# kmkolasinski/tfrecords-reader

Hardware: AMD Instinct MI355X
Metric: GiB/s + examples/s device-resident TFRecord->Feature decode, 1/2/4/8 GPU (higher is better)
Workload: dtype u8; 1 GPU; C4 directory (configs[4]) of 256 files, C1-shaped (int64 label + 12 B bytes_list id) records, 524288 +-50 % per file (default_rng(1000+f)), spec CRC-32C; this rank's LPT share (256 files) resident in HBM; records_per_gpu=134295581, framed_bytes_per_gpu=7906235019, parallelism=file-sharded x1 (LPT by bytes, no collective on the data path), batches_per_gpu=4, batch_bytes_max=1976558779, streams=2, tpl_groups_missed=0

## Files before the change

### tfrecords-reader_amd/csrc/tfrg_capi.cpp

```cpp
#include <hip/hip_runtime.h>
#include <stdlib.h>
#include <string.h>

#include <algorithm>
#include <map>
#include <numeric>
#include <string>
#include <unordered_map>
#include <vector>

#include "../../include/tfrg.h"
#include "crc32c.h"
#include "tfrg_internal.h"

namespace tfrg {
void set_error(const std::string& s);

#define HIP_TRY(expr)                                                              \
  do {                                                                             \
    hipError_t e_ = (expr);                                                        \
    if (e_ != hipSuccess) {                                                        \
      set_error(std::string(#expr) + ": " + hipGetErrorString(e_));               \
      return TFRG_E_HIP;                                                           \
    }                                                                              \
// ... 12 lines not shown
    }
    size_t want = bytes < 256 ? 256 : bytes;
    want = (want + 4095) & ~(size_t)4095;
    hipError_t e = hipMalloc(&p, want);
    if (e == hipSuccess) cap = want;
    return e;
  }
  void release() {
    if (p) (void)hipFree(p);
    p = nullptr;
    cap = 0;
  }
  template <class T>
  T* as() const {
    return reinterpret_cast<T*>(p);
  }
};

constexpr uint32_t kMissCap = 1u << 16;

const CrcTables& crc_tables() {
  static const CrcTables T = [] {
    CrcTables t;
    crc_make_tables(&t);
    return t;
  }();
  return T;
}

}

using namespace tfrg;

struct Offsets {
  const uint64_t* s64 = nullptr;
  const uint64_t* e64 = nullptr;
  const uint32_t* s32 = nullptr;
  const uint32_t* e32 = nullptr;
  uint32_t first = 0;
  uint32_t mode = kOffU64;
};

struct tfrg_ctx {
  int device = 0;
  hipStream_t own_stream = nullptr;
  hipStream_t last_stream = nullptr;
  uint32_t lane_max = 2048;
  uint32_t wave_stage = 0xffffffffu;
  uint64_t record_bound = 0;
  uint64_t call_bound = 0;
  int num_cus = 256;
  uint32_t cu_lds = 65536;
  int tpl_stage = 1;
  DBuf crc_tab, consts;
  DBuf ht, key_hash, key_off, key_blob, key_slot, slot_kind, key_w, krec;
  uint32_t n_keys = 0, n_slots = 0, ht_mask = 0;
  DBuf in_bytes, in_start, in_end;
  DBuf status, aux, verdict, order, count, loc, rs, slot_base, totals, kind_totals;
  DBuf ident;
  size_t ident_n = 0;
  DBuf i64, f32, b_off, b_len, big_list, slow_list, miss, info, tsum, crc_rec, crc_base, crc_part;
  DBuf dq, dq_cnt;
  DBuf lmask, rlist;
  DBuf bdata, boff64, blb, bbig;
  bool materialized = false;
  bool tsum_dirty = true;
  uint32_t info_slot = 0;
  bool info_clean = false;
  uint32_t n = 0;
  uint64_t cap_hint = 0;
  hipEvent_t order_ev = nullptr;
  uint64_t nbytes = 0;
  uint64_t cap_i64 = 0, cap_f32 = 0, cap_b = 0;
  bool have_result = false;
  bool rs_complete = false;
  std::unordered_map<std::string, uint32_t> key_id;
  std::vector<int32_t> key_slot_h;
  DBuf tpl;
  uint32_t n_tpl = 0;
  uint32_t tpl_w = 0;
  size_t tpl_img_off = 0;
  uint32_t tpl_img_words = 0;
  uint32_t tpl_tab_words = 0;
  std::vector<uint32_t> tpl_h;
  bool tpl_learned = false;
  bool tpl_full = false;
  uint32_t tpl_frames = 0;
  bool tpl_on = true;
  std::vector<uint8_t> slot_kind_h;
  DBuf spec;
  std::vector<uint32_t> spec_h;
  bool have_spec = false;
  bool spec_on = true;
  bool profiling = false;
  bool have_events = false;
  hipEvent_t ev[kNumStages + 1] = {};
  uint64_t hint_i64 = 0, hint_f32 = 0, hint_b = 0;
  bool hinted = false;
  bool no_hints = false;
  uint64_t hint_reruns = 0;
  bool optimistic_on = true;
  bool walk_beside = true;
  uint32_t walk_blocks = 0;
  bool no_quiet = false;
  bool opt_pending = false;
  bool ord_const = false;
  bool len_const = false;
  std::vector<uint32_t> const_len;
  uint32_t last_implicit = 0;
  bool last_aux_zero = false;
  uint32_t* info_pin = nullptr;
  bool cols_complete = false;
  bool mat_pending = false;
  struct LastCall {
    const uint8_t* d_bytes;
    uint64_t nbytes;
    uint64_t cap_in;
    uint64_t bound;
    uint32_t n, flags;
    hipStream_t st;
  } last{};
  Offsets last_off{};
  uint32_t poison[4] = {0xffffffffu, 0xffffffffu, 0xffffffffu, 0xffffffffu};
};

extern "C" {

int tfrg_ctx_create(int device, tfrg_ctx** out) {
  *out = nullptr;
  int ndev = 0;
  HIP_TRY(hipGetDeviceCount(&ndev));
  if (device < 0 || device >= ndev) {
    set_error("bad device index");
    return TFRG_E_ARG;
  }
  HIP_TRY(hipSetDevice(device));
  tfrg_ctx* c = new tfrg_ctx();
  c->device = device;
  if (const char* e = getenv("TFRG_TEMPLATES")) c->tpl_on = atoi(e) != 0;
  if (const char* e = getenv("TFRG_SPEC")) c->spec_on = atoi(e) != 0;
  if (const char* e = getenv("TFRG_TPL_STAGE")) c->tpl_stage = atoi(e);
  if (const char* e = getenv("TFRG_OPTIMISTIC")) c->optimistic_on = atoi(e) != 0;
  if (const char* e = getenv("TFRG_WALK_BESIDE")) c->walk_beside = atoi(e) != 0;
  if (const char* e = getenv("TFRG_WALK_BLOCKS")) c->walk_blocks = (uint32_t)atoi(e);
  if (const char* e = getenv("TFRG_DEBUG_POISON_LOC")) {
    char* q = const_cast<char*>(e);
    for (int i = 0; i < 4 && *q; ++i) {
      c->poison[i] = (uint32_t)strtoul(q, &q, 10);
      while (*q == ',' || *q == ' ') ++q;
    }
  }
  hipDeviceProp_t prop;
  if (hipGetDeviceProperties(&prop, device) == hipSuccess) {
    c->num_cus = prop.multiProcessorCount;
    if (prop.maxSharedMemoryPerMultiProcessor) c->cu_lds = (uint32_t)prop.maxSharedMemoryPerMultiProcessor;
  }
  if (hipStreamCreateWithFlags(&c->own_stream, hipStreamNonBlocking) != hipSuccess) {
    delete c;
    set_error("hipStreamCreate failed");
    return TFRG_E_HIP;
  }
  if (hipHostMalloc(reinterpret_cast<void**>(&c->info_pin), (kInfoCount + 8) * 4) != hipSuccess) {
    (void)hipStreamDestroy(c->own_stream);
    delete c;
    set_error("hipHostMalloc failed");
    return TFRG_E_NOMEM;
  }
  std::vector<uint32_t> tab(kCrcTabWords), cst(128);
  CrcTables T;
  crc_make_tables(&T);
  memcpy(tab.data(), T.t, 4096);
  uint32_t M[4][256];
  crc_make_mul_tables(gf_xpow8(1024), M);
  memcpy(tab.data() + 1024, M, 4096);
  memcpy(tab.data() + 2048, T.t, 8192);
  memcpy(tab.data() + 4096, T.t, 16384);
  for (int e = 0; e < 256; ++e)
    for (int col = 0; col < 47; ++col) tab[8192 + e * 64 + col] = T.t[(col + 1) & 15][e];
  crc_make_mul_tables(gf_xpow8(2048), M);
  memcpy(tab.data() + 24576, M, 4096);
  crc_make_mul_tables(gf_xpow8(4096), M);
  memcpy(tab.data() + 25600, M, 4096);
  for (int k = 0; k < 24; ++k) {
    crc_make_mul_tables(gf_xpow8(1024ull << k), M);
    memcpy(tab.data() + 26624 + k * 1024, M, 4096);
  }
  for (int l = 0; l < 64; ++l) cst[l] = gf_xpow8(16ull * l);
  for (int z = 0; z < 16; ++z) cst[64 + z] = gf_xpow8_inv((uint64_t)z);
  for (int k = 0; k < 32; ++k) cst[96 + k] = gf_xpow8(1024ull << k);
  if (c->crc_tab.ensure(tab.size() * 4) != hipSuccess || c->consts.ensure(cst.size() * 4) != hipSuccess ||
      hipMemcpy(c->crc_tab.p, tab.data(), tab.size() * 4, hipMemcpyHostToDevice) != hipSuccess ||
      hipMemcpy(c->consts.p, cst.data(), cst.size() * 4, hipMemcpyHostToDevice) != hipSuccess) {
    set_error("constant upload failed");
    tfrg_ctx_destroy(c);
// ... 837 lines not shown
    if (!n) HIP_TRY(hipMemsetAsync(c->boff64.p, 0, 8, st));
  }
  if (!S || !n) HIP_TRY(hipMemsetAsync(c->kind_totals.p, 0, 32, st));

  DevBatch b;
  b.bytes = d_bytes;
  b.nbytes = nbytes;
  b.start = off.s64;
  b.end = off.e64;
  b.start32 = off.s32;
  b.end32 = off.e32;
  b.first = off.first;
  b.omode = off.mode;
  b.n = n;
  b.flags = flags;
  DevOut o;
  o.status = c->status.as<int32_t>();
  o.aux = c->aux.as<int64_t>();
  o.verdict = c->verdict.as<uint8_t>();
  o.order = c->order.as<uint16_t>();
  o.count = c->count.as<uint32_t>();
  o.loc = c->loc.as<uint2>();
  o.rs = c->rs.as<uint32_t>();
  o.slot_base = c->slot_base.as<uint64_t>();
  o.totals = c->totals.as<uint32_t>();
  o.kind_totals = c->kind_totals.as<uint64_t>();
  o.i64 = c->i64.as<int64_t>();
  o.f32 = c->f32.as<uint32_t>();
  o.b_off = c->b_off.as<uint32_t>();
  o.b_len = c->b_len.as<uint32_t>();
  o.cap_i64 = cap_i64;
  o.cap_f32 = cap_f32;
  o.cap_b = cap_b;
  o.big_list = c->big_list.as<uint32_t>();
  o.miss = c->miss.as<uint32_t>();
  o.miss_cap = kMissCap;
  o.info = info_cur;
  o.info_next = c->info.as<uint32_t>() + (islot ^ 1u) * kInfoCount;
  o.tsum = c->tsum.as<uint32_t>();
  o.tile_stride = tile_stride;
  o.spine_lb = reinterpret_cast<uint64_t*>(o.tsum + (size_t)S * tile_stride);
  o.n_chunks = n_chunks;
  o.irr = o.tsum + (size_t)S * tile_stride + 2ull * S * n_chunks;
  o.slow_list = c->slow_list.as<uint32_t>();
  o.crc_rec = c->crc_rec.as<uint32_t>();
  o.crc_base = c->crc_base.as<uint64_t>();
  o.crc_part = c->crc_part.as<uint64_t>();
  o.lmask = c->lmask.as<uint64_t>();
  o.rlist = c->rlist.as<uint32_t>();
  LaunchCfg cfg;
  cfg.num_cus = c->num_cus;
  cfg.tpl_cu_lds = c->tpl_stage ? c->cu_lds : 0u;
  cfg.tpl_stage_any = c->tpl_stage == 2;
  cfg.lean = c->tpl_on && c->n_tpl;
  cfg.tpl_full = cfg.lean && c->tpl_full;
  cfg.tpl_unchecked = cfg.lean && (c->tpl_frames & 2u) != 0;
  cfg.spec_h = c->spec_h.empty() ? nullptr : c->spec_h.data();
  const uint64_t lane_blocks = (n + 255) / 256;
  const uint64_t lane_cap = (uint64_t)c->num_cus * 8;
  cfg.lane_grid = (int)(lane_blocks < 1 ? 1 : (lane_blocks < lane_cap ? lane_blocks : lane_cap));
  const uint64_t wave_cap = (uint64_t)c->num_cus * 4;
  const uint64_t wave_blocks = (n + 3) / 4;
  cfg.wave_grid = (int)(wave_blocks < 1 ? 1 : (wave_blocks < wave_cap ? wave_blocks : wave_cap));
  cfg.lane_max = c->lane_max;
  cfg.wave_stage = c->wave_stage;
  memcpy(cfg.poison, c->poison, sizeof(cfg.poison));
  cfg.optimistic = c->optimistic_on && !c->no_quiet && c->poison[0] == 0xffffffffu;
  cfg.walk_beside = c->walk_beside;
  cfg.walk_blocks = c->walk_blocks;
  cfg.ran_optimistic = false;
  cfg.ran_quiet_big = false;
  cfg.ord_const = c->ord_const;
  cfg.len_const = c->len_const && !mat;
  cfg.implicit = 0;
  const uint64_t bound = c->call_bound ? c->call_bound : c->record_bound;
  c->call_bound = 0;
  c->last = tfrg_ctx::LastCall{d_bytes, nbytes, cap_in, bound, n, flags, st};
  c->last_off = off;
  o.dq = nullptr;
  o.dq_cnt = nullptr;
  o.dq_blocks = 0;
  cfg.body_count = false;
  if (n && (bound == 0 || bound > c->lane_max)) {
    uint64_t blocks = nbytes >> 18;
    blocks = blocks < 16 ? 16 : (blocks > (1u << 16) ? (1u << 16) : blocks);
    const size_t qb = (size_t)blocks * 64u * kDeferK * 16u, cb = (size_t)blocks * 64u;
    if ((c->dq.cap < qb || c->dq_cnt.cap < cb) && c->last_stream) HIP_TRY(hipStreamSynchronize(c->last_stream));
    if (c->dq.ensure(qb) || c->dq_cnt.ensure(cb)) {
      set_error("device allocation failed (deferred bodies)");
      return TFRG_E_NOMEM;
    }
    o.dq = c->dq.as<uint4>();
    o.dq_cnt = c->dq_cnt.as<uint8_t>();
    o.dq_blocks = (uint32_t)blocks;
    cfg.body_count = true;
  }
  if (n) {
    hipEvent_t* ev = nullptr;
    if (c->profiling) {
      if (!c->have_events) {
        for (auto& e : c->ev) HIP_TRY(hipEventCreate(&e));
        c->have_events = true;
      }
      ev = c->ev;
    }
    hipError_t e = launch_decode(b, schema_view(c), o, cfg, c->crc_tab.as<uint32_t>(), c->consts.as<uint32_t>(), st, ev);
// ... 280 lines not shown
```

### tfrecords-reader_amd/csrc/tfrg_internal.h

```cpp
#pragma once
#include <stdint.h>
#include <hip/hip_runtime.h>

namespace tfrg {

struct DevSchema {
  uint32_t n_keys;
  uint32_t n_slots;
  uint32_t ht_mask;
  const uint32_t* ht;
  const uint32_t* key_hash;
  const uint32_t* key_off;
  const uint8_t* key_blob;
  const int32_t* key_slot;
  const uint8_t* slot_kind;
  const uint32_t* key_w;
  const uint32_t* krec;
  const uint32_t* tpl;
  const uint32_t* tpl_img;
  uint32_t tpl_img_words;
  uint32_t tpl_tab_words;
  uint32_t n_tpl;
  uint32_t tpl_w;
  const uint32_t* spec;
};

constexpr uint32_t kTplMaxL = 240, kTplMaxEntries = 16;
constexpr uint32_t kLtMaxW = 64;
constexpr uint32_t kLeanMaxSlots = 16;
constexpr uint32_t kLtL = 0, kLtNe = 1, kLtCrcw = 2, kLtChain = 3, kLtK = 4, kLtAbsent = 5, kLtFrame = 6, kLtEnt = 8,
                   kLtWin = kLtEnt + 4 * kTplMaxEntries, kLtSlot = kLtWin + 3 * kLtMaxW,
                   kLtWords = kLtSlot + 3 * kLeanMaxSlots;
constexpr uint32_t kCrcTabWords = 51200;

constexpr uint32_t kLiPtabWords = 4 * 256;
constexpr uint32_t kTplMaxLane = 32;
constexpr uint32_t kLiHdr = 8, kLiSlotQ = kLiHdr, kLiLut = kLiSlotQ + kLeanMaxSlots,
                   kLiLutWords = (kTplMaxL + 1 + 3) / 4, kLiTpl = (kLiLut + kLiLutWords + 3) & ~3u;
constexpr uint32_t kLiQValue = 1u << 16, kLiQSingle = 1u << 17;
__host__ __device__ constexpr uint32_t kLiTw(uint32_t W) { return 4 + 3 * W + 4 * kLeanMaxSlots; }
constexpr uint32_t kLiMaxWords = (65536u - 32768u - 512u) / 4u;

struct LeanTgt {
  uint16_t* ord;
  uint32_t* cnt;
  uint2* loc;
  uint32_t* rs;
  void* v1;
  uint32_t* v2;
  uint32_t lim;
  uint32_t kind;
  uint32_t pad[2];
};
struct LeanArgs {
  uint32_t n_tpl;
  uint32_t lane_max;
  uint32_t* tsum;
  uint32_t n_slots;
  uint32_t tile_stride;
  uint32_t img_words;
  uint32_t gpw;
  uint32_t bsplit;
  uint32_t gsplit;
  const uint8_t* finish;
  uint32_t implicit;
  uint32_t tab_words;
  uint32_t cu_lds;
  uint32_t stage_any;
  uint32_t nocrc;
  uint32_t strict;
  uint32_t uframes;
  LeanTgt tg[kLeanMaxSlots];
};

enum KeyRec : uint32_t { kKrHash = 0, kKrLen, kKrW0, kKrW1, kKrSlot1, kKrSlot2, kKrSlot3, kKrFlags, kKrWords };
constexpr uint32_t kLdsMaxKeys = 256;
constexpr uint32_t kLdsMaxHt = 1024;

__host__ __device__ inline uint32_t key_hash_words(uint32_t n, uint32_t w0, uint32_t w1) {
  const uint32_t a = (w0 ^ (w0 >> 11) ^ (n << 17)) & 0xffffffu;
  const uint32_t b = (w1 ^ (w1 >> 13) ^ (n << 7)) & 0xffffffu;
#if defined(__HIP_DEVICE_COMPILE__)
  uint32_t p0, p1;
  asm("v_mul_u32_u24 %0, %1, %2" : "=v"(p0) : "v"(a), "v"(0x9E3779u));
  asm("v_mul_u32_u24 %0, %1, %2" : "=v"(p1) : "v"(b), "v"(0x85EBCBu));
  uint32_t h = p0 ^ p1;
#else
  uint32_t h = a * 0x9E3779u;
  h ^= b * 0x85EBCBu;
#endif
  return h ^ (h >> 15);
}

enum OffMode : uint32_t { kOffU64 = 0, kOffU32 = 1, kOffEnds = 2 };

struct DevBatch {
  const uint8_t* bytes;
  uint64_t nbytes;
  const uint64_t* start;
  const uint64_t* end;
  const uint32_t* start32;
  const uint32_t* end32;
  uint32_t first;
  uint32_t omode;
  uint32_t n;
  uint32_t flags;
};

#if defined(__HIPCC__)
__device__ __forceinline__ uint64_t rec_end(const DevBatch& B, uint32_t r) {
  return B.omode == kOffU64 ? B.end[r] : (uint64_t)B.end32[r];
}
__device__ __forceinline__ uint64_t rec_start(const DevBatch& B, uint32_t r) {
  if (B.omode == kOffU64) return B.start[r];
  if (B.omode == kOffU32) return B.start32[r];
  return r ? (uint64_t)B.end32[r - 1] : (uint64_t)B.first;
}
#endif

enum InfoIdx : uint32_t {
  kInfoErrors = 0,
// ... 70 lines not shown
  uint64_t* lmask;
  uint32_t* rlist;
};

constexpr uint32_t kTileShift = 8;
constexpr uint32_t kTileRecs = 1u << kTileShift;
constexpr uint32_t kSpineChunkShift = 12;

constexpr uint32_t kFlagPayloadOnly = 1u;
constexpr uint32_t kFlagSpecVarint = 2u;
constexpr uint32_t kFlagNoCrc = 4u;
constexpr uint32_t kFlagStrictCrc = 8u;
constexpr uint32_t kFlagMaterializeBytes = 16u;


struct DevBytes {
  const uint8_t* in;
  uint64_t in_readable;
  const uint32_t* b_off;
  const uint32_t* b_len;
  const uint64_t* kind_totals;
  uint64_t* offsets;
  uint64_t offsets_cap;
  uint8_t* data;
  uint64_t data_cap;
  uint64_t* lb;
  uint32_t* ticket;
  uint32_t* big_count;
  uint32_t* big_list;
  uint32_t* overflow;
};
hipError_t launch_materialize(const DevBytes& d, int num_cus, hipStream_t st);
uint64_t materialize_lb_words(uint64_t cap_b);

struct LaunchCfg {
  int num_cus;
  bool lean;
  bool tpl_full;
  bool tpl_unchecked;
  const uint32_t* spec_h;
  int lane_grid;
  int wave_grid;
  uint32_t lane_max;
  uint32_t wave_stage;
  bool body_count;
  uint32_t poison[4];
  bool optimistic;
  bool ran_optimistic;
  bool ord_const;
  bool len_const;
  bool ran_quiet_big;
  uint32_t tpl_cu_lds;
  bool tpl_stage_any;
  bool walk_beside;
  uint32_t walk_blocks;
  uint32_t implicit;
};

enum Stage : int { kStageTplLane = 0, kStageLaneCount, kStageBodyCount, kStageTailCount, kStageSpine,
                   kStageDownGather, kStageTailGather, kStageMaterialize, kNumStages };
extern const char* const kStageNames[kNumStages];

hipError_t launch_tpl_lane(const DevBatch& b, const DevOut& o, const LeanArgs& a, const uint32_t* img, uint32_t w,
                           int num_cus, hipStream_t st);
hipError_t launch_fill_placed_rows(uint32_t* rs, const uint32_t* info, uint32_t n_slots, uint32_t n, hipStream_t st);
hipError_t launch_stream_read(const void* d, uint64_t nbytes, uint32_t* sink, hipStream_t st, int variant);
hipError_t launch_decode(const DevBatch& b, const DevSchema& sc, const DevOut& o, LaunchCfg& cfg,
                         const uint32_t* d_crc_tables, const uint32_t* d_wave_consts, hipStream_t stream,
                         hipEvent_t* ev);

}
```

### tfrecords-reader_amd/csrc/tfrg_kernels.hip

```cpp
#include <hip/hip_runtime.h>
#include <algorithm>
#include <type_traits>
#include "tfrg_internal.h"
#include "crc32c.h"
#include "tfrg_walk.h"
#include "../../include/tfrg_status.h"

namespace tfrg {

#ifdef TFRG_PHASE_PROF
__device__ unsigned long long g_phase[32];
#define PHASE_MARK(t) const uint64_t t = __builtin_readcyclecounter()
#define PHASE_ADD(i, a, b) \
  do {                     \
    if (lane == 0) atomicAdd(&g_phase[i], (unsigned long long)((b) - (a))); \
  } while (0)
#else
#define PHASE_MARK(t) (void)0
#define PHASE_ADD(i, a, b) (void)0
#endif

struct Src {
  const uint8_t* buf;
  uint64_t p0;
// ... 3083 lines not shown

template <bool COMPAT>
static hipError_t launch_all(const DevBatch& b, const DevSchema& sc, const DevOut& o, LaunchCfg& cfg,
                             const uint32_t* d_tab, const uint32_t* d_consts, hipStream_t st, hipEvent_t* ev) {
  auto mark = [&](int i) {
    if (ev) (void)hipEventRecord(ev[i], st);
  };
  const size_t S = sc.n_slots;
  const uint32_t n_tiles = (b.n + kTileRecs - 1) / kTileRecs;
  const size_t dict_lane = S * kLaneCountBlock * 4 + r16(S * kLaneCountBlock * 2);
  const size_t tab_lds = 256ull * kLaneSlice * kLaneRep * 4;
  const size_t stage_lds = (size_t)kStageStride * (kLaneCountBlock / 64);
  const bool fast_ok = sc.n_keys <= kLdsMaxKeys && sc.ht_mask + 1 <= kLdsMaxHt;
  const size_t keys_lds = fast_ok ? (((size_t)sc.ht_mask + 4) / 4 * 4 + (size_t)sc.n_keys * kKrWords) * 4 : 0;
  const size_t spec_lds = fast_ok && sc.spec ? ((S + 7) & ~(size_t)7) * 4 + S * kSpecTgtWords * 4 : 0;
  const size_t lane_lds = tab_lds + dict_lane + stage_lds + keys_lds + spec_lds;
  DevSchema scx = sc;
  if (lane_lds > kLaneLdsBudget || !fast_ok) scx.spec = nullptr;
  const uint32_t wave_stage = cfg.wave_stage < kWStage ? cfg.wave_stage : kWStage;
  const bool lean = cfg.lean && sc.n_tpl && fast_ok && S <= kLeanMaxSlots && o.lmask && o.rlist &&
                    (sc.tpl_w == 16 || sc.tpl_w == 32 || sc.tpl_w == 64) &&
                    !(b.flags & kFlagPayloadOnly) && b.nbytes < 0xffffff00ull;
  const bool tpl_nocrc = (b.flags & kFlagNoCrc) != 0, tpl_strict = (b.flags & kFlagStrictCrc) != 0;
  const bool quiet = lean && cfg.tpl_full && !cfg.body_count;
  bool all_spec = scx.spec && cfg.spec_h && S <= 64;
  for (size_t k = 0; all_spec && k < S; ++k) all_spec = cfg.spec_h[k] != 0u;
  cfg.ran_optimistic = cfg.optimistic && quiet && all_spec && S > 0 && !(tpl_strict && cfg.tpl_unchecked);
  const bool quiet_big = cfg.optimistic && !lean && all_spec && S > 0 && lane_lds <= kLaneLdsBudget && fast_ok &&
                         cfg.body_count && !(b.flags & kFlagStrictCrc) && b.n > 0;
  cfg.ran_optimistic |= quiet_big;
  cfg.ran_quiet_big = quiet_big;
  const size_t slow_tail = 2048ull * 4 + S * kTailBlock * 4 + r16(S * kTailBlock * 2);
  const bool tail_gord = slow_tail > kLaneLdsBudget;
  const size_t tail_lds = std::max<size_t>(tail_gord ? 2048ull * 4 : slow_tail, (kTailFinishWord + 4) * 4);
  const size_t walk_lds = 256ull * kLaneSlice * 4 + S * kTailBlock * 4 + r16(S * kTailBlock * 2) + keys_lds + spec_lds;
  const bool walk_beside = quiet_big && cfg.walk_beside && walk_lds <= tail_lds;
  cfg.implicit = 0;
  DevOut ox = o;
  if (!lean) {
    ox.lmask = nullptr;
    ox.rlist = nullptr;
  }
  mark(kStageTplLane);
  if (lean) {
    LeanArgs a{};
    a.n_tpl = sc.n_tpl;
    a.img_words = sc.tpl_img_words;
    a.tab_words = tpl_nocrc ? 0u : sc.tpl_tab_words;
    a.nocrc = tpl_nocrc ? 1u : 0u;
    a.strict = tpl_strict ? 1u : 0u;
    a.uframes = cfg.tpl_unchecked ? 1u : 0u;
    a.cu_lds = cfg.tpl_cu_lds;
    a.stage_any = cfg.tpl_stage_any ? 1u : 0u;
    a.lane_max = cfg.lane_max;
    a.tsum = cfg.ran_optimistic ? nullptr : o.tsum;
    a.finish = cfg.ran_optimistic ? sc.slot_kind : nullptr;
    cfg.implicit = cfg.ran_optimistic ? (!tpl_nocrc && !cfg.tpl_unchecked ? TFRG_IMPLICIT_STATUS : 0u) |
                                            (cfg.ord_const ? TFRG_IMPLICIT_ORDER : 0u) |
                                            (cfg.len_const ? TFRG_IMPLICIT_BYTES_LEN : 0u)
                                      : 0u;
    a.implicit = cfg.implicit;
    a.n_slots = (uint32_t)S;
    a.tile_stride = o.tile_stride;
    const uint64_t n = b.n;
    for (uint32_t k = 0; k < S; ++k) {
      LeanTgt& t = a.tg[k];
      t.ord = o.order + k * n;
      t.cnt = o.count + k * n;
      t.loc = o.loc + k * n;
      t.rs = o.rs + k * (n + 1);
      const uint32_t sw = scx.spec && cfg.spec_h ? cfg.spec_h[k] : 0u;
      if (sw) {
        const uint32_t kind = sw & 3u;
        const uint64_t base = n * ((sw >> 2) - 1u);
        const uint64_t cap = kind == TFRG_KIND_INT64 ? o.cap_i64 : kind == TFRG_KIND_FLOAT ? o.cap_f32 : o.cap_b;
        t.lim = cap > base ? (uint32_t)std::min<uint64_t>(cap - base, n) : 0u;
        t.kind = kind;
        if (kind == TFRG_KIND_INT64) t.v1 = o.i64 + base;
        else if (kind == TFRG_KIND_FLOAT) t.v1 = o.f32 + base;
        else t.v1 = o.b_off + base;
        t.v2 = o.b_len + base;
      }
    }
    const hipError_t e = launch_tpl_lane(b, ox, a, sc.tpl_img, sc.tpl_w, cfg.num_cus, st);
    if (e != hipSuccess) return e;
  }
  if (cfg.ran_optimistic && !quiet_big) {
    for (int i = kStageLaneCount; i <= kStageMaterialize; ++i) mark(i);
    return hipGetLastError();
  }
  mark(kStageLaneCount);
  auto resident_grid = [&](const void* fn, size_t lds, bool cap = true) {
    int per_cu = 0;
    if (hipOccupancyMaxActiveBlocksPerMultiprocessor(&per_cu, fn, kLaneCountBlock, lds) != hipSuccess || per_cu < 1)
      per_cu = 1;
    const int g = per_cu * cfg.num_cus;
    int need = (int)(((int64_t)cfg.lane_grid * 256 + kLaneCountBlock - 1) / kLaneCountBlock);
    if (quiet) need = std::min(need, 64);
    return g < need || !cap ? g : need;
  };
  if (lane_lds <= kLaneLdsBudget) {
    const void* fn = reinterpret_cast<const void*>(&k_lane_count<kLaneRep, COMPAT, 0>);
    hipLaunchKernelGGL((k_lane_count<kLaneRep, COMPAT, 0>), dim3(resident_grid(fn, lane_lds - tab_lds)),
                       dim3(kLaneCountBlock), lane_lds - tab_lds, st, b, scx, ox, d_tab, cfg.lane_max, wave_stage,
                       walk_beside ? 1u : 0u);
  } else if (S <= 64) {
// ... 157 lines not shown
```

### tfrecords-reader_amd/csrc/tfrg_tpl.hip

```cpp
#include <hip/hip_runtime.h>
#include "tfrg_internal.h"
#include "crc32c.h"
#include "../../include/tfrg_status.h"

namespace tfrg {

namespace {

constexpr int kTplBlock = 512;
constexpr uint32_t kTplTabWords = 8;
static_assert(4u * kTplTabWords * kLiPtabWords + 4u * kLiMaxWords + 512u <= 65536u, "lane image + CRC tables exceed LDS");
constexpr uint32_t kStageWords = 1024 + 32, kStageRounds = (kStageWords * 4u + 1023u) / 1024u;
constexpr uint32_t kHitVerdict = TFRG_V_LEN_MATCH | TFRG_V_LEN_CRC | TFRG_V_DATA_CRC;

typedef __attribute__((address_space(4))) const uint32_t cu32;

__device__ __forceinline__ uint32_t rfl(uint32_t x) { return __builtin_amdgcn_readfirstlane(x); }

template <int K>
__device__ __forceinline__ uint32_t bx4(uint32_t x) {
  uint32_t r;
  const uint32_t two = 2u;
  if constexpr (K == 0)
    asm("v_lshlrev_b32_sdwa %0, %1, %2 dst_sel:DWORD dst_unused:UNUSED_PAD src0_sel:DWORD src1_sel:BYTE_0"
        : "=v"(r) : "v"(two), "v"(x));
  else if constexpr (K == 1)
    asm("v_lshlrev_b32_sdwa %0, %1, %2 dst_sel:DWORD dst_unused:UNUSED_PAD src0_sel:DWORD src1_sel:BYTE_1"
        : "=v"(r) : "v"(two), "v"(x));
  else if constexpr (K == 2)
    asm("v_lshlrev_b32_sdwa %0, %1, %2 dst_sel:DWORD dst_unused:UNUSED_PAD src0_sel:DWORD src1_sel:BYTE_2"
        : "=v"(r) : "v"(two), "v"(x));
  else
    asm("v_lshlrev_b32_sdwa %0, %1, %2 dst_sel:DWORD dst_unused:UNUSED_PAD src0_sel:DWORD src1_sel:BYTE_3"
        : "=v"(r) : "v"(two), "v"(x));
  return r;
}

__device__ __forceinline__ uint32_t xor3(uint32_t a, uint32_t b, uint32_t c) {
  return __builtin_amdgcn_bitop3_b32(a, b, c, 0x96);
}

template <int Q>
__device__ __forceinline__ uint32_t tl(const uint8_t* tw, uint32_t bx) {
  return *reinterpret_cast<const uint32_t*>(tw + Q * 1024 + bx);
}

__device__ __forceinline__ uint32_t lin_word(const uint8_t* tw, uint32_t x) {
  return xor3(tl<3>(tw, bx4<0>(x)), tl<2>(tw, bx4<1>(x)), tl<1>(tw, bx4<2>(x))) ^ tl<0>(tw, bx4<3>(x));
}

__device__ __forceinline__ uint32_t vgroups(uint32_t w, uint32_t m) {
  w &= m;
  return (w & 0x7fu) | ((w >> 1) & 0x3f80u) | ((w >> 2) & 0x1fc000u) | ((w >> 3) & 0xfe00000u);
}
__device__ __forceinline__ uint32_t bytes_mask(uint32_t nb) { return nb >= 4u ? 0xffffffffu : (1u << (nb << 3)) - 1u; }

typedef uint32_t u32x4 __attribute__((ext_vector_type(4)));

struct LaneOff {
  uint32_t s, e;
};

__device__ __forceinline__ uint32_t wave_sum(uint32_t x) {
#pragma unroll
  for (int m = 1; m < 64; m <<= 1) x += (uint32_t)__shfl_xor((int)x, m, 64);
  return x;
}

__device__ void tpl_quiet_finish(const DevOut& o, const uint8_t* slot_kind, uint32_t n_slots, uint32_t n,
                                 uint32_t listed) {
  if (threadIdx.x < kInfoCount) o.info_next[threadIdx.x] = 0u;
  if (listed != 0u) return;
  for (uint32_t k = threadIdx.x; k < n_slots; k += kTplBlock) {
    o.totals[k] = n;
    o.rs[(size_t)k * (n + 1u) + n] = n;
  }
  if (threadIdx.x == 0) {
    uint64_t acc[4] = {0, 0, 0, 0};
    for (uint32_t k = 0; k < n_slots; ++k) {
      const uint32_t kd = slot_kind[k] & 3u;
      o.slot_base[k] = acc[kd];
      acc[kd] += n;
    }
    for (int k = 0; k < 4; ++k) o.kind_totals[k] = acc[k];
    if (acc[TFRG_KIND_INT64] > o.cap_i64 || acc[TFRG_KIND_FLOAT] > o.cap_f32 || acc[TFRG_KIND_BYTES] > o.cap_b)
      o.info[kInfoOverflow] = 1u;
    const uint64_t pm = n_slots >= 64u ? ~0ull : (1ull << n_slots) - 1ull;
    o.info[kInfoPlacedLo] = (uint32_t)pm;
    o.info[kInfoPlacedHi] = (uint32_t)(pm >> 32);
  }
}

template <int W, int OM, bool ST, bool UF>
__global__ __launch_bounds__(kTplBlock, W == 16 ? 6 : (W == 32 ? 4 : 2)) void k_tpl_lane(
    DevBatch B, DevOut o, LeanArgs A, const uint32_t* __restrict__ img, const uint32_t* __restrict__ tabs) {
  static_assert(W == 16 || W == 32 || W == 64, "window words");
  static_assert(!ST || W == 16, "staged windows: W = 16");
  typedef uint32_t wvec __attribute__((ext_vector_type(W)));
  extern __shared__ __attribute__((aligned(16))) uint32_t tab[];
  uint32_t* const limg = tab + A.tab_words;
  constexpr uint32_t kWaves = kTplBlock / 64;
  constexpr uint32_t kTw = kLiTw(W);
  const uint32_t lane = threadIdx.x & 63u, wib = rfl(threadIdx.x >> 6);
  cu32* gimg = (cu32*)img;
  const bool nocrc = UF && A.nocrc;
  const uint32_t crcw_u = nocrc ? 0u : gimg[3], chain_u = nocrc ? (uint32_t)W : gimg[4];
  auto tabw = [&](uint32_t j) -> const uint8_t* {
    return reinterpret_cast<const uint8_t*>(tab) + 4u * kLiPtabWords * ((gimg[6u + (j >> 2)] >> (8u * (j & 3u))) & 0xffu);
  };
  const uint8_t* lut = reinterpret_cast<const uint8_t*>(limg + kLiLut);
  const __amdgpu_buffer_rsrc_t rsrc =
      __builtin_amdgcn_make_buffer_rsrc(const_cast<uint8_t*>(B.bytes), (short)0, (int)(uint32_t)B.nbytes, 0x00020000);
  const uint32_t nb = (uint32_t)B.nbytes;
  const uint32_t ngroups = (B.n + 63u) >> 6;
  static_assert(kTileShift == 8, "4 groups of 64 records per tile");
  const bool tail = blockIdx.x >= A.bsplit;
  const uint32_t gpw = tail ? 2u : A.gpw;
  const uint32_t gbeg0 = tail ? A.gsplit + ((blockIdx.x - A.bsplit) * kWaves + wib) * 2u : (blockIdx.x * kWaves + wib) * gpw;
  const uint32_t gbeg = gbeg0 < ngroups ? gbeg0 : ngroups;
  const uint32_t gend = gbeg + gpw < ngroups ? gbeg + gpw : ngroups;
  const bool whole = (gpw & 3u) == 0u;

  auto offsets = [&](uint32_t g) -> LaneOff {
    LaneOff f{1u, 0u};
    const uint32_t r = (g << 6) + lane;
    if (g < gend && r < B.n) {
      if constexpr (OM == kOffU64) {
        const uint64_t s = B.start[r], e = B.end[r];
        if (((s | e) >> 32) == 0) f = LaneOff{(uint32_t)s, (uint32_t)e};
      } else if constexpr (OM == kOffU32) {
        f = LaneOff{B.start32[r], B.end32[r]};
      } else {
        f.e = B.end32[r];
        f.s = lane ? 0u : (r ? B.end32[r - 1] : B.first);
      }
    }
    return f;
  };
  auto start_of = [&](const LaneOff& f) -> uint32_t {
    if constexpr (OM == kOffEnds)
      return (uint32_t)__builtin_amdgcn_update_dpp((int)f.s, (int)f.e, 0x138, 0xf, 0xf, false);
    else
      return f.s;
  };
  auto in_batch = [&](uint32_t g, uint32_t s, uint32_t e) {
    return (g << 6) + lane < B.n && s <= e && e <= nb && e >= 16u;
  };
  auto window = [&](wvec& wn, const LaneOff& f) {
    const uint32_t e = f.e;
    const bool full = e >= 4u * W && e <= nb;
    const uint32_t voff = full ? e - 4u * W : 0xffffff00u;
#pragma unroll
    for (int q = 0; q < W / 4; ++q) {
      const u32x4 v = __builtin_bit_cast(u32x4, __builtin_amdgcn_raw_buffer_load_b128(rsrc, voff + 16u * q, 0, 0));
      wn[4 * q] = v.x;
      wn[4 * q + 1] = v.y;
      wn[4 * q + 2] = v.z;
      wn[4 * q + 3] = v.w;
    }
  };
  auto window_st = [&](wvec& wn, const LaneOff& f, uint32_t g) {
    if constexpr (ST) {
      uint32_t* const stg = limg + A.img_words + wib * kStageWords;
      const uint32_t e = f.e;
      const uint32_t g0 = g << 6;
      const uint32_t nv = g < gend ? (B.n - g0 < 64u ? B.n - g0 : 64u) : 0u;
      const uint32_t pe = (uint32_t)__builtin_amdgcn_update_dpp((int)e, (int)e, 0x138, 0xf, 0xf, false);
      const bool bad = lane < nv && (e < pe || e > nb);
      if (nv && !__ballot(bad)) {
        const uint32_t e0 = rfl(e), hi = (uint32_t)__builtin_amdgcn_readlane((int)e, (int)(nv - 1u));
        const uint32_t lo = (e0 >= 4u * W ? e0 - 4u * W : 0u) & ~15u;
        const uint32_t nch = (hi - lo + 15u) >> 4;
        if (hi > lo && nch * 16u + 4u <= kStageWords * 4u && lo + nch * 16u <= nb) {
          u32x4 t[kStageRounds];
#pragma unroll
          for (uint32_t k = 0; k < kStageRounds; ++k)
            if (lane + 64u * k < nch)
              t[k] = __builtin_bit_cast(u32x4, __builtin_amdgcn_raw_buffer_load_b128(rsrc, lo + 16u * (lane + 64u * k), 0, 0));
#pragma unroll
          for (uint32_t k = 0; k < kStageRounds; ++k)
            if (lane + 64u * k < nch) reinterpret_cast<u32x4*>(stg)[lane + 64u * k] = t[k];
          __builtin_amdgcn_wave_barrier();
          const bool full = e >= 4u * W && lane < nv;
          const uint32_t b0 = full ? e - 4u * W - lo : 0u;
          const uint32_t* const sp = stg + (b0 >> 2);
          const uint32_t sh = b0 & 3u;
          uint32_t prev = sp[0];
#pragma unroll
          for (int i = 0; i < W; ++i) {
            const uint32_t nx = sp[i + 1];
            wn[i] = __builtin_amdgcn_alignbyte(nx, prev, sh);
            prev = nx;
          }
          __builtin_amdgcn_wave_barrier();
          if (__ballot(!full)) {
#pragma unroll
            for (int i = 0; i < W; ++i) wn[i] = full ? wn[i] : 0u;
          }
          return;
        }
      }
    }
    window(wn, f);
  };
  auto head_fix = [&](wvec& wn, const LaneOff& f, uint32_t g) {
    if (g != 0u) return;
    const uint32_t e = f.e;
    const bool full = e >= 4u * W && e <= nb;
    const bool head = in_batch(g, start_of(f), e) && !full;
    if (__ballot(head)) {
#pragma unroll
      for (int i = 0; i < W; ++i) {
        uint32_t x = 0;
#pragma unroll
        for (int b = 0; b < 4; ++b) {
          const int64_t p = (int64_t)e - 4 * W + 4 * i + b;
          if (head && p >= 0) x |= (uint32_t)__builtin_amdgcn_raw_buffer_load_b8(rsrc, (uint32_t)p, 0, 0) << (8 * b);
        }
        if (head) wn[i] = x;
      }
    }
  };
  auto wsel = [](const wvec& w, uint32_t q) -> uint32_t {
    if constexpr (W <= 32) {
      return w[q & (W - 1u)];
    } else {
      uint32_t a = 0;
#pragma unroll
      for (int i = 0; i < W; ++i)
        if (q == (uint32_t)i) a = w[i];
      return a;
    }
  };
  uint32_t acc = 0;
  uint32_t listed = 0;
  auto proc = [&](const wvec& w, uint32_t g, const LaneOff& f) {
    const uint32_t r = (g << 6) + lane;
    const bool valid = r < B.n;
    const uint32_t st = start_of(f), en = f.e;
    const bool inb = in_batch(g, st, en);
    const uint32_t rl = en - st;
    uint32_t cand = inb && rl >= 16u && rl - 16u <= kTplMaxL && rl <= A.lane_max ? (uint32_t)lut[rl - 16u] : 0xffu;
    uint32_t tsel = 0xffu;
    while (__ballot(cand != 0xffu)) {
      const bool act = cand != 0xffu;
      const uint32_t* tp = limg + kLiTpl + (act ? cand : 0u) * kTw;
      const u32x4 meta = *reinterpret_cast<const u32x4*>(tp);
      uint32_t diff = 0;
#pragma unroll
      for (int q = 0; q < W / 4; ++q) {
        const u32x4 bm = *reinterpret_cast<const u32x4*>(tp + 4 + 4 * q);
        const u32x4 mm = *reinterpret_cast<const u32x4*>(tp + 4 + W + 4 * q);
        diff |= ((w[4 * q] ^ bm.x) & mm.x) | ((w[4 * q + 1] ^ bm.y) & mm.y) | ((w[4 * q + 2] ^ bm.z) & mm.z) |
                ((w[4 * q + 3] ^ bm.w) & mm.w);
        if (q & 1) __builtin_amdgcn_sched_barrier(0);
      }
      const uint32_t* cm = tp + 4 + 2 * W;
      uint32_t c = 0;
      if (chain_u < (uint32_t)(W - 9)) {
#pragma unroll
        for (int i = 0; i < W - 9; ++i)
          if ((uint32_t)i >= chain_u) c = lin_word(tabw(7), c ^ (w[i] & cm[i]));
      }
      uint32_t lin = 0;
#define TFRG_LIN(j)                                                                                       \
  if (crcw_u & (1u << (j))) lin ^= lin_word(tabw(j), (w[W - 9 + (j)] & cm[W - 9 + (j)]) ^ ((j) == 0 ? c : 0u));
      TFRG_LIN(0) TFRG_LIN(1) TFRG_LIN(2) TFRG_LIN(3) TFRG_LIN(4) TFRG_LIN(5) TFRG_LIN(6) TFRG_LIN(7)
#undef TFRG_LIN
      bool ok = act && diff == 0u;
      if constexpr (UF) {
        const uint32_t mc = crc_mask(lin ^ meta.y);
        ok = ok && (nocrc || (meta.w ? mc != 0u && !A.strict : mc == w[W - 1]));
      } else {
        ok = ok && crc_mask(lin ^ meta.y) == w[W - 1];
      }
      tsel = ok ? cand : tsel;
      cand = act && !ok ? meta.z : 0xffu;
    }
    const bool hit = tsel != 0xffu;
    if (hit && !(A.implicit & TFRG_IMPLICIT_STATUS)) {
      o.status[r] = TFRG_OK;
      if constexpr (UF)
        o.verdict[r] = (uint8_t)(nocrc || limg[kLiTpl + tsel * kTw + 3] ? (uint32_t)TFRG_V_LEN_MATCH : kHitVerdict);
      else
        o.verdict[r] = (uint8_t)kHitVerdict;
    }
    if (__ballot(hit)) {
      const uint32_t* ts = limg + kLiTpl + (hit ? tsel : 0u) * kTw + 4 + 3 * W;
      for (uint32_t k = 0; k < A.n_slots; ++k) {
        const uint32_t sq = gimg[kLiSlotQ + k];
        const u32x4 z = *reinterpret_cast<const u32x4*>(ts + 4u * k);
        const uint32_t mode = z.x & 0xffu, len = (z.x >> 8) & 0xffu, pos = z.y, cw = z.z;
        uint32_t lx = pos, ly = len;
        if (sq & kLiQValue) {
          const uint32_t qw = pos >> 2;
          uint32_t a = 0, b = 0;
          for (uint32_t i = sq & 0xffu; i <= ((sq >> 8) & 0xffu); ++i) {
            const bool at = qw == i;
            a = at ? wsel(w, i) : a;
            b = at ? wsel(w, i + 1u) : b;
          }
          const uint32_t x = __builtin_amdgcn_alignbyte(b, a, pos & 3u);
          if (mode == 1u || mode == 2u) {
            lx = mode == 1u ? vgroups(x, bytes_mask(len)) : x;
            ly = 0;
          }
        }
        if (mode == 3u) lx = en + pos;
        const uint32_t tot = !A.tsum ? 0u
                             : (sq & kLiQSingle) ? (uint32_t)__popcll(__ballot(hit && cw != 0u))
                                                 : wave_sum(hit ? (cw & ~kCountInline) : 0u);
        const LeanTgt& T = A.tg[k];
        if (hit) {
          if (!(A.implicit & TFRG_IMPLICIT_ORDER)) T.ord[r] = (uint16_t)(z.x >> 16);
          if (T.kind) {
            if (r < T.lim) {
              if (T.kind == TFRG_KIND_INT64) {
                reinterpret_cast<uint64_t*>(T.v1)[r] = lx;
              } else {
                reinterpret_cast<uint32_t*>(T.v1)[r] = lx;
                if (T.kind == TFRG_KIND_BYTES && !(A.implicit & TFRG_IMPLICIT_BYTES_LEN)) T.v2[r] = ly;
              }
            }
          } else {
            T.cnt[r] = cw;
            T.loc[r] = make_uint2(lx, ly);
          }
        }
        acc += lane == k ? tot : 0u;
      }
    }
    const uint64_t mm = __ballot(valid && !hit);
    if (lane == 0) {
      o.lmask[g] = mm;
      if (mm) o.rlist[atomicAdd(&o.info[kInfoResid], 1u)] = g;
    }
    listed += mm ? 1u : 0u;
  };
  auto flush = [&](uint32_t g) {
    if (lane < A.n_slots && acc && A.tsum) {
      if (whole)
        A.tsum[lane * A.tile_stride + (g >> 2)] = acc;
      else
        atomicAdd(&A.tsum[lane * A.tile_stride + (g >> 2)], acc);
    }
    acc = 0;
  };
  LaneOff fa = offsets(gbeg), f0 = offsets(gbeg + 1u);
  static_assert(kTplTabWords * kLiPtabWords % (4u * kTplBlock) == 0u, "table copy in whole 16-byte rounds");
  constexpr uint32_t kTabRounds = kTplTabWords * kLiPtabWords / (4u * kTplBlock);
  const uint32_t tab16 = A.tab_words >> 2;
  u32x4 tv[kTabRounds];
#pragma unroll
  for (uint32_t j = 0; j < kTabRounds; ++j)
    if (threadIdx.x + j * kTplBlock < tab16) tv[j] = reinterpret_cast<const u32x4*>(tabs)[threadIdx.x + j * kTplBlock];
  const uint32_t iw0 = threadIdx.x < A.img_words ? img[threadIdx.x] : 0u;
  wvec wa;
  window_st(wa, fa, gbeg);
#pragma unroll
  for (uint32_t j = 0; j < kTabRounds; ++j)
    if (threadIdx.x + j * kTplBlock < tab16) reinterpret_cast<u32x4*>(tab)[threadIdx.x + j * kTplBlock] = tv[j];
  if (threadIdx.x < A.img_words) limg[threadIdx.x] = iw0;
  for (uint32_t i = threadIdx.x + kTplBlock; i < A.img_words; i += kTplBlock) limg[i] = img[i];
  __syncthreads();
  for (uint32_t g = gbeg; g < gend; ++g) {
    head_fix(wa, fa, g);
    proc(wa, g, fa);
    if (((g + 1u) & 3u) == 0u || g + 1u >= gend) flush(g);
    if (g + 1u < gend) {
      window_st(wa, f0, g + 1u);
      fa = f0;
      f0 = offsets(g + 2u);
    }
  }
  if (A.finish) {
    __shared__ uint32_t s_listed[kWaves];
    __shared__ uint32_t s_last, s_total;
    if (lane == 0) s_listed[wib] = listed;
    __syncthreads();
    if (threadIdx.x == 0) {
      uint32_t mine = 0;
      for (uint32_t i = 0; i < kWaves; ++i) mine += s_listed[i];
      const uint64_t old = atomicAdd(reinterpret_cast<unsigned long long*>(o.info + kInfoTplDone),
                                     ((unsigned long long)mine << 32) | 1ull);
      s_last = (uint32_t)old == gridDim.x - 1u;
      s_total = (uint32_t)(old >> 32) + mine;
    }
    __syncthreads();
    if (s_last) tpl_quiet_finish(o, A.finish, A.n_slots, B.n, s_total);
  }
}

}

hipError_t launch_tpl_lane(const DevBatch& b, const DevOut& o, const LeanArgs& a, const uint32_t* img, uint32_t w,
                           int num_cus, hipStream_t st) {
  const uint32_t groups = (b.n + 63u) / 64u;
  const uint32_t tiles = (groups + 3u) / 4u;
  const uint32_t need = (tiles + kTplBlock / 64 - 1) / (kTplBlock / 64);
  LeanArgs a2 = a;
  a2.gpw = need < (uint32_t)num_cus / 2u ? 1u : need < (uint32_t)num_cus ? 2u : need >= 8u * (uint32_t)num_cus ? 8u : 4u;
  static const bool split_on = [] {
    const char* e = getenv("TFRG_TPL_TAIL");
    return !e || atoi(e) != 0;
  }();
  constexpr uint32_t kW = kTplBlock / 64;
  uint32_t gsplit = groups, bsplit = 0xffffffffu;
  if (split_on && a2.gpw == 8u) {
    const uint32_t small = 3u * (uint32_t)num_cus * kW * 2u;
    if (groups > 4u * small) {
      const uint32_t big_blocks = (groups - small) / (kW * a2.gpw);
      gsplit = big_blocks * kW * a2.gpw;
      bsplit = big_blocks;
    }
  }
  a2.gsplit = gsplit;
  a2.bsplit = bsplit;
  const uint32_t blocks = bsplit != 0xffffffffu
                              ? bsplit + (groups - gsplit + kW * 2u - 1u) / (kW * 2u)
                              : ((groups + a2.gpw - 1u) / a2.gpw + kW - 1u) / kW;
  const dim3 grid(blocks ? blocks : 1u);
  const uint32_t* tabs = img + a.img_words;
  size_t lds = ((size_t)a.tab_words + a.img_words) * 4;
  const size_t lds_st = lds + (size_t)kW * kStageWords * 4;
  const bool staged = w == 16 && (a2.gpw >= 8u || a.stage_any) && lds_st + 64u <= 65536u &&
                      3u * ((lds_st + 64u + 2047u) & ~(size_t)2047u) <= a.cu_lds;
  if (staged) lds = lds_st;
  const bool uf = a.nocrc || a.uframes;
#define TFRG_TPL_LAUNCH(WW, OO, SS)                                                                            \
  if (uf) hipLaunchKernelGGL((k_tpl_lane<WW, OO, SS, true>), grid, dim3(kTplBlock), lds, st, b, o, a2, img, tabs); \
  else hipLaunchKernelGGL((k_tpl_lane<WW, OO, SS, false>), grid, dim3(kTplBlock), lds, st, b, o, a2, img, tabs)
#define TFRG_TPL_OM(WW, SS)                                                    \
  switch (b.omode) {                                                           \
    case kOffU64: TFRG_TPL_LAUNCH(WW, kOffU64, SS); break;                     \
    case kOffU32: TFRG_TPL_LAUNCH(WW, kOffU32, SS); break;                     \
    default: TFRG_TPL_LAUNCH(WW, kOffEnds, SS); break;                         \
  }
  switch (w) {
    case 16:
      if (staged) {
        TFRG_TPL_OM(16, true)
      } else {
        TFRG_TPL_OM(16, false)
      }
      break;
    case 32: TFRG_TPL_OM(32, false) break;
    case 64: TFRG_TPL_OM(64, false) break;
    default: return hipErrorInvalidValue;
  }
#undef TFRG_TPL_OM
#undef TFRG_TPL_LAUNCH
  return hipGetLastError();
}

}
```

Before: 4155 GiB/s.

## Stage template windows via async buffer-to-LDS loads and nontemporal output stores

In the staged template-lane kernel, window bytes now go straight from global memory to static LDS through buffer_load_lds. The load for the next group is issued before the current group is processed, and explicit waitcnt calls overlap the load with compute instead of round-tripping through registers. Output stores on the staged path use nontemporal stores. The LDS layout moves from dynamic to fixed static arrays. A TFRG_TPL_GPW env knob is added to force groups-per-wave. The hand-written waitcnt encodings and static LDS sizing add correctness and occupancy risk.

```diff
diff --git a/tfrecords-reader_amd/csrc/tfrg_capi.cpp b/tfrecords-reader_amd/csrc/tfrg_capi.cpp
--- a/tfrecords-reader_amd/csrc/tfrg_capi.cpp
+++ b/tfrecords-reader_amd/csrc/tfrg_capi.cpp
@@ -88,6 +88,7 @@
   int num_cus = 256;
   uint32_t cu_lds = 65536;
   int tpl_stage = 1;
+  uint32_t tpl_gpw = 0;
   DBuf crc_tab, consts;
   DBuf ht, key_hash, key_off, key_blob, key_slot, slot_kind, key_w, krec;
   uint32_t n_keys = 0, n_slots = 0, ht_mask = 0;
@@ -176,6 +177,10 @@
   if (const char* e = getenv("TFRG_TEMPLATES")) c->tpl_on = atoi(e) != 0;
   if (const char* e = getenv("TFRG_SPEC")) c->spec_on = atoi(e) != 0;
   if (const char* e = getenv("TFRG_TPL_STAGE")) c->tpl_stage = atoi(e);
+  if (const char* e = getenv("TFRG_TPL_GPW")) {
+    const int v = atoi(e);
+    if (v == 2 || v == 4 || v == 8) c->tpl_gpw = (uint32_t)v;
+  }
   if (const char* e = getenv("TFRG_OPTIMISTIC")) c->optimistic_on = atoi(e) != 0;
   if (const char* e = getenv("TFRG_WALK_BESIDE")) c->walk_beside = atoi(e) != 0;
   if (const char* e = getenv("TFRG_WALK_BLOCKS")) c->walk_blocks = (uint32_t)atoi(e);
@@ -1119,6 +1124,7 @@
   cfg.num_cus = c->num_cus;
   cfg.tpl_cu_lds = c->tpl_stage ? c->cu_lds : 0u;
   cfg.tpl_stage_any = c->tpl_stage == 2;
+  cfg.tpl_gpw = c->tpl_gpw;
   cfg.lean = c->tpl_on && c->n_tpl;
   cfg.tpl_full = cfg.lean && c->tpl_full;
   cfg.tpl_unchecked = cfg.lean && (c->tpl_frames & 2u) != 0;
diff --git a/tfrecords-reader_amd/csrc/tfrg_internal.h b/tfrecords-reader_amd/csrc/tfrg_internal.h
--- a/tfrecords-reader_amd/csrc/tfrg_internal.h
+++ b/tfrecords-reader_amd/csrc/tfrg_internal.h
@@ -67,6 +67,7 @@
   uint32_t tab_words;
   uint32_t cu_lds;
   uint32_t stage_any;
+  uint32_t gpw_force;
   uint32_t nocrc;
   uint32_t strict;
   uint32_t uframes;
@@ -243,6 +244,7 @@
   bool ran_quiet_big;
   uint32_t tpl_cu_lds;
   bool tpl_stage_any;
+  uint32_t tpl_gpw;
   bool walk_beside;
   uint32_t walk_blocks;
   uint32_t implicit;
diff --git a/tfrecords-reader_amd/csrc/tfrg_kernels.hip b/tfrecords-reader_amd/csrc/tfrg_kernels.hip
--- a/tfrecords-reader_amd/csrc/tfrg_kernels.hip
+++ b/tfrecords-reader_amd/csrc/tfrg_kernels.hip
@@ -3159,6 +3159,7 @@
     a.uframes = cfg.tpl_unchecked ? 1u : 0u;
     a.cu_lds = cfg.tpl_cu_lds;
     a.stage_any = cfg.tpl_stage_any ? 1u : 0u;
+    a.gpw_force = cfg.tpl_gpw;
     a.lane_max = cfg.lane_max;
     a.tsum = cfg.ran_optimistic ? nullptr : o.tsum;
     a.finish = cfg.ran_optimistic ? sc.slot_kind : nullptr;
diff --git a/tfrecords-reader_amd/csrc/tfrg_tpl.hip b/tfrecords-reader_amd/csrc/tfrg_tpl.hip
--- a/tfrecords-reader_amd/csrc/tfrg_tpl.hip
+++ b/tfrecords-reader_amd/csrc/tfrg_tpl.hip
@@ -11,9 +11,42 @@
 constexpr uint32_t kTplTabWords = 8;
 static_assert(4u * kTplTabWords * kLiPtabWords + 4u * kLiMaxWords + 512u <= 65536u, "lane image + CRC tables exceed LDS");
 constexpr uint32_t kStageWords = 1024 + 32, kStageRounds = (kStageWords * 4u + 1023u) / 1024u;
+constexpr uint32_t kStTimgWords = (53248u - 64u - (kTplBlock / 64u) * kStageWords * 4u) / 16u * 4u;
+template <bool ST>
+__device__ __forceinline__ uint32_t* st_timg() {
+  if constexpr (ST) {
+    __shared__ __attribute__((aligned(16))) uint32_t s_timg[kStTimgWords];
+    return s_timg;
+  } else {
+    return nullptr;
+  }
+}
+template <bool ST>
+__device__ __forceinline__ uint32_t* st_stage() {
+  if constexpr (ST) {
+    __shared__ __attribute__((aligned(16))) uint32_t s_stage[(kTplBlock / 64u) * kStageWords];
+    return s_stage;
+  } else {
+    return nullptr;
+  }
+}
 constexpr uint32_t kHitVerdict = TFRG_V_LEN_MATCH | TFRG_V_LEN_CRC | TFRG_V_DATA_CRC;
 
 typedef __attribute__((address_space(4))) const uint32_t cu32;
+typedef __attribute__((address_space(3))) void lds_void;
+#ifndef TFRG_TPL_SPAN_AUX
+#define TFRG_TPL_SPAN_AUX 2
+#endif
+#ifndef TFRG_TPL_STORE_NT
+#define TFRG_TPL_STORE_NT 1
+#endif
+template <bool NT, typename T>
+__device__ __forceinline__ void put(T* p, T v) {
+  if constexpr (NT)
+    __builtin_nontemporal_store(v, p);
+  else
+    *p = v;
+}
 
 __device__ __forceinline__ uint32_t rfl(uint32_t x) { return __builtin_amdgcn_readfirstlane(x); }
 
@@ -97,7 +130,9 @@
   static_assert(W == 16 || W == 32 || W == 64, "window words");
   static_assert(!ST || W == 16, "staged windows: W = 16");
   typedef uint32_t wvec __attribute__((ext_vector_type(W)));
-  extern __shared__ __attribute__((aligned(16))) uint32_t tab[];
+  extern __shared__ __attribute__((aligned(16))) uint32_t dyn_lds[];
+  uint32_t* tab = dyn_lds;
+  if constexpr (ST) tab = st_timg<ST>();
   uint32_t* const limg = tab + A.tab_words;
   constexpr uint32_t kWaves = kTplBlock / 64;
   constexpr uint32_t kTw = kLiTw(W);
@@ -159,9 +194,13 @@
       wn[4 * q + 3] = v.w;
     }
   };
-  auto window_st = [&](wvec& wn, const LaneOff& f, uint32_t g) {
+  struct Span {
+    uint32_t lo;
+    bool on;
+  };
+  auto fill = [&](const LaneOff& f, uint32_t g) -> Span {
     if constexpr (ST) {
-      uint32_t* const stg = limg + A.img_words + wib * kStageWords;
+      uint32_t* const stg = st_stage<ST>() + wib * kStageWords;
       const uint32_t e = f.e;
       const uint32_t g0 = g << 6;
       const uint32_t nv = g < gend ? (B.n - g0 < 64u ? B.n - g0 : 64u) : 0u;
@@ -172,36 +211,42 @@
         const uint32_t lo = (e0 >= 4u * W ? e0 - 4u * W : 0u) & ~15u;
         const uint32_t nch = (hi - lo + 15u) >> 4;
         if (hi > lo && nch * 16u + 4u <= kStageWords * 4u && lo + nch * 16u <= nb) {
-          u32x4 t[kStageRounds];
 #pragma unroll
           for (uint32_t k = 0; k < kStageRounds; ++k)
             if (lane + 64u * k < nch)
-              t[k] = __builtin_bit_cast(u32x4, __builtin_amdgcn_raw_buffer_load_b128(rsrc, lo + 16u * (lane + 64u * k), 0, 0));
-#pragma unroll
-          for (uint32_t k = 0; k < kStageRounds; ++k)
-            if (lane + 64u * k < nch) reinterpret_cast<u32x4*>(stg)[lane + 64u * k] = t[k];
-          __builtin_amdgcn_wave_barrier();
-          const bool full = e >= 4u * W && lane < nv;
-          const uint32_t b0 = full ? e - 4u * W - lo : 0u;
-          const uint32_t* const sp = stg + (b0 >> 2);
-          const uint32_t sh = b0 & 3u;
-          uint32_t prev = sp[0];
-#pragma unroll
-          for (int i = 0; i < W; ++i) {
-            const uint32_t nx = sp[i + 1];
-            wn[i] = __builtin_amdgcn_alignbyte(nx, prev, sh);
-            prev = nx;
-          }
-          __builtin_amdgcn_wave_barrier();
-          if (__ballot(!full)) {
-#pragma unroll
-            for (int i = 0; i < W; ++i) wn[i] = full ? wn[i] : 0u;
-          }
-          return;
+              __builtin_amdgcn_raw_ptr_buffer_load_lds(rsrc, (lds_void*)(stg + 256u * k), 16, lo + 16u * (lane + 64u * k), 0,
+                                                       0, TFRG_TPL_SPAN_AUX);
+          return Span{lo, true};
         }
       }
     }
+    return Span{0u, false};
+  };
+  auto take = [&](wvec& wn, const LaneOff& f, uint32_t g, const Span& sp_) {
+    if constexpr (ST) {
+      if (sp_.on) {
+        const uint32_t* const stg = st_stage<ST>() + wib * kStageWords;
+        const uint32_t e = f.e;
+        const bool full = e >= 4u * W && (g << 6) + lane < B.n;
+        const uint32_t b0 = full ? e - 4u * W - sp_.lo : 0u;
+        const uint32_t* const sp = stg + (b0 >> 2);
+        const uint32_t sh = b0 & 3u;
+        uint32_t prev = sp[0];
+#pragma unroll
+        for (int i = 0; i < W; ++i) {
+          const uint32_t nx = sp[i + 1];
+          wn[i] = __builtin_amdgcn_alignbyte(nx, prev, sh);
+          prev = nx;
+        }
+        if (__ballot(!full)) {
+#pragma unroll
+          for (int i = 0; i < W; ++i) wn[i] = full ? wn[i] : 0u;
+        }
+        return;
+      }
+    }
     window(wn, f);
+    if constexpr (ST) __builtin_amdgcn_s_waitcnt(0x0F70);
   };
   auto head_fix = [&](wvec& wn, const LaneOff& f, uint32_t g) {
     if (g != 0u) return;
@@ -219,6 +264,7 @@
         }
         if (head) wn[i] = x;
       }
+      if constexpr (ST) __builtin_amdgcn_s_waitcnt(0x0F70);
     }
   };
   auto wsel = [](const wvec& w, uint32_t q) -> uint32_t {
@@ -315,11 +361,12 @@
           if (!(A.implicit & TFRG_IMPLICIT_ORDER)) T.ord[r] = (uint16_t)(z.x >> 16);
           if (T.kind) {
             if (r < T.lim) {
+              constexpr bool kNt = ST && TFRG_TPL_STORE_NT;
               if (T.kind == TFRG_KIND_INT64) {
-                reinterpret_cast<uint64_t*>(T.v1)[r] = lx;
+                put<kNt>(reinterpret_cast<uint64_t*>(T.v1) + r, (uint64_t)lx);
               } else {
-                reinterpret_cast<uint32_t*>(T.v1)[r] = lx;
-                if (T.kind == TFRG_KIND_BYTES && !(A.implicit & TFRG_IMPLICIT_BYTES_LEN)) T.v2[r] = ly;
+                put<kNt>(reinterpret_cast<uint32_t*>(T.v1) + r, lx);
+                if (T.kind == TFRG_KIND_BYTES && !(A.implicit & TFRG_IMPLICIT_BYTES_LEN)) put<kNt>(T.v2 + r, ly);
               }
             }
           } else {
@@ -356,21 +403,46 @@
     if (threadIdx.x + j * kTplBlock < tab16) tv[j] = reinterpret_cast<const u32x4*>(tabs)[threadIdx.x + j * kTplBlock];
   const uint32_t iw0 = threadIdx.x < A.img_words ? img[threadIdx.x] : 0u;
   wvec wa;
-  window_st(wa, fa, gbeg);
+  Span sa{0u, false};
+  if constexpr (ST)
+    sa = fill(fa, gbeg);
+  else
+    window(wa, fa);
 #pragma unroll
   for (uint32_t j = 0; j < kTabRounds; ++j)
     if (threadIdx.x + j * kTplBlock < tab16) reinterpret_cast<u32x4*>(tab)[threadIdx.x + j * kTplBlock] = tv[j];
   if (threadIdx.x < A.img_words) limg[threadIdx.x] = iw0;
   for (uint32_t i = threadIdx.x + kTplBlock; i < A.img_words; i += kTplBlock) limg[i] = img[i];
   __syncthreads();
-  for (uint32_t g = gbeg; g < gend; ++g) {
-    head_fix(wa, fa, g);
-    proc(wa, g, fa);
-    if (((g + 1u) & 3u) == 0u || g + 1u >= gend) flush(g);
-    if (g + 1u < gend) {
-      window_st(wa, f0, g + 1u);
+  if constexpr (ST) {
+    for (uint32_t g = gbeg; g < gend; ++g) {
+      asm volatile("" ::: "memory");
+      __builtin_amdgcn_s_waitcnt(0x0F70);
+      asm volatile("" ::: "memory");
+      take(wa, fa, g, sa);
+      asm volatile("" ::: "memory");
+      __builtin_amdgcn_s_waitcnt(0xC07F);
+      asm volatile("" ::: "memory");
+      Span sn{0u, false};
+      if (g + 1u < gend) sn = fill(f0, g + 1u);
+      const LaneOff f2 = offsets(g + 2u);
+      head_fix(wa, fa, g);
+      proc(wa, g, fa);
+      if (((g + 1u) & 3u) == 0u || g + 1u >= gend) flush(g);
       fa = f0;
-      f0 = offsets(g + 2u);
+      f0 = f2;
+      sa = sn;
+    }
+  } else {
+    for (uint32_t g = gbeg; g < gend; ++g) {
+      head_fix(wa, fa, g);
+      proc(wa, g, fa);
+      if (((g + 1u) & 3u) == 0u || g + 1u >= gend) flush(g);
+      if (g + 1u < gend) {
+        window(wa, f0);
+        fa = f0;
+        f0 = offsets(g + 2u);
+      }
     }
   }
   if (A.finish) {
@@ -400,13 +472,15 @@
   const uint32_t need = (tiles + kTplBlock / 64 - 1) / (kTplBlock / 64);
   LeanArgs a2 = a;
   a2.gpw = need < (uint32_t)num_cus / 2u ? 1u : need < (uint32_t)num_cus ? 2u : need >= 8u * (uint32_t)num_cus ? 8u : 4u;
+  const bool forced = a.gpw_force == 2u || a.gpw_force == 4u || a.gpw_force == 8u;
+  if (forced) a2.gpw = a.gpw_force;
   static const bool split_on = [] {
     const char* e = getenv("TFRG_TPL_TAIL");
     return !e || atoi(e) != 0;
   }();
   constexpr uint32_t kW = kTplBlock / 64;
   uint32_t gsplit = groups, bsplit = 0xffffffffu;
-  if (split_on && a2.gpw == 8u) {
+  if (split_on && !forced && a2.gpw == 8u) {
     const uint32_t small = 3u * (uint32_t)num_cus * kW * 2u;
     if (groups > 4u * small) {
       const uint32_t big_blocks = (groups - small) / (kW * a2.gpw);
@@ -422,10 +496,11 @@
   const dim3 grid(blocks ? blocks : 1u);
   const uint32_t* tabs = img + a.img_words;
   size_t lds = ((size_t)a.tab_words + a.img_words) * 4;
-  const size_t lds_st = lds + (size_t)kW * kStageWords * 4;
-  const bool staged = w == 16 && (a2.gpw >= 8u || a.stage_any) && lds_st + 64u <= 65536u &&
+  constexpr size_t lds_st = ((size_t)kStTimgWords + kW * kStageWords) * 4;
+  static_assert(lds_st + 64u <= 65536u, "staged kernel's LDS");
+  const bool staged = w == 16 && (a2.gpw >= 8u || a.stage_any) && (size_t)a.tab_words + a.img_words <= kStTimgWords &&
                       3u * ((lds_st + 64u + 2047u) & ~(size_t)2047u) <= a.cu_lds;
-  if (staged) lds = lds_st;
+  if (staged) lds = 0;
   const bool uf = a.nocrc || a.uframes;
 #define TFRG_TPL_LAUNCH(WW, OO, SS)                                                                            \
   if (uf) hipLaunchKernelGGL((k_tpl_lane<WW, OO, SS, true>), grid, dim3(kTplBlock), lds, st, b, o, a2, img, tabs); \
```

New measurement: 4456 GiB/s (median of 6 runs). 7.2% higher.
